# yugabyte/yugabyte-db

Hardware: NVIDIA H100
Metric: compaction GB/s (input bytes merged) (higher is better)
Workload: dtype u8

## Files before the change

yugabyte-db_b200/csrc/engine.cu:

```cuda
#include "engine.h"
#include "host_sst.h"

#include <cuda_runtime.h>
#include <algorithm>
#include <cstdio>
#include <cstring>
#include <chrono>
#include <cstdlib>
#include <mutex>

namespace ybgpu {

#define CUDA_TRY(expr)                                                                      \
  do {                                                                                      \
    cudaError_t _e = (expr);                                                                \
    if (_e != cudaSuccess) {                                                                \
      return FailCuda(#expr, _e);                                                           \
    }                                                                                       \
  } while (0)

struct RunView {
  const uint8_t* data;
  const uint64_t* blk_off;
  const uint32_t* blk_size;
// ... 15 lines not shown
struct JobDev {
  int error;
  uint32_t error_where;
  uint32_t max_ikey_len;
  uint32_t restart_interval[MAX_RUNS];
  unsigned long long in_key_bytes, in_val_bytes;
  unsigned long long n_counted, n_hidden, n_obsolete, n_feed_dropped, n_kept, out_key_bytes, out_val_bytes;
  unsigned long long min_seq, max_seq, n_kept_deletions;
  uint32_t n_rewrites;
  uint32_t n_tiles;
  uint32_t max_tile;
  int ingest_fallback;
  uint32_t n_compressed;
  uint32_t n_lz4;
  uint32_t n_cont_tiles;
  unsigned long long digest;
  unsigned long long verify_fail;
};

struct JobParams {
  int S;
  int k;
  int bottommost;
  uint64_t last_sequence;
  uint32_t largest_len; uint8_t largest[1024];
  uint32_t tile_cap;
  uint32_t H;
  uint32_t M;
  RetentionDev R;
  RangeDev range;
};

struct Desc {
  uint32_t gid;
  uint32_t vlen_out;
  uint16_t klen;
  uint8_t flags;
  uint8_t run;
  uint32_t rewrite_slot;
};

__device__ __forceinline__ void dev_fail(JobDev* J, int code, uint32_t where) {
  if (atomicCAS(&J->error, 0, code) == 0) J->error_where = where;
}

__device__ __forceinline__ uint32_t ldg_u32_unaligned(const uint8_t* p) {
  return static_cast<uint32_t>(p[0]) | (static_cast<uint32_t>(p[1]) << 8) | (static_cast<uint32_t>(p[2]) << 16) |
         (static_cast<uint32_t>(p[3]) << 24);
}

__global__ void __launch_bounds__(256) k_prepass(const RunView* runs, const uint32_t* blk_base , int k, JobDev* J) {
  const int lane = threadIdx.x & 31;
  const uint32_t warp = (blockIdx.x * blockDim.x + threadIdx.x) >> 5;
  const uint32_t nwarps = (gridDim.x * blockDim.x) >> 5;
  unsigned long long key_bytes = 0, val_bytes = 0;
  uint32_t max_klen = 0;
  const uint32_t total_blocks = blk_base[k];
  for (uint32_t gb = warp; gb < total_blocks; gb += nwarps) {
// ... 314 lines not shown
        run.val_off[idx] = boff + p;
        p += vlen;
        idx++;
      }
    }
  }
}

struct PartView {
  const RunView* runs;
  const uint32_t* sample_base;
  uint32_t* pos;
  unsigned long long* bucket_min;
  uint8_t* smode;
  uint32_t n_samples;
  uint32_t n_buckets;
};

constexpr unsigned long long TILE_CONT = 1ull << 63;
constexpr uint32_t SAMPLE_COARSE = 32;
__global__ void __launch_bounds__(256) k_sample_pos(PartView P, const JobParams* prm, JobDev* J, int pass) {
  const int S = prm->S, k = prm->k;
  const uint64_t total = static_cast<uint64_t>(P.n_samples) * k;
  for (uint64_t t = blockIdx.x * static_cast<uint64_t>(blockDim.x) + threadIdx.x; t < total;
       t += static_cast<uint64_t>(gridDim.x) * blockDim.x) {
    const uint32_t s = static_cast<uint32_t>(t / k), r2 = static_cast<uint32_t>(t % k);
    int r = 0;
    while (r + 1 < k && P.sample_base[r + 1] <= s) r++;
    const uint32_t s_local = s - P.sample_base[r];
    if (((s_local % SAMPLE_COARSE) == 0) != (pass == 0)) continue;
    const uint32_t idx = s_local * prm->M;
    const uint8_t* srec = P.runs[r].rec + static_cast<size_t>(idx) * S;
    const int g = group_prefix_len(srec, rec_ulen(srec, S), prm->R.enabled != 0);
    if (g < 0) { dev_fail(J, -g, s); continue; }
    bool inside = false;
    if (idx >= prm->M) {
      const uint8_t* prec = srec - static_cast<size_t>(prm->M) * S;
      inside = rec_ulen(prec, S) >= static_cast<uint32_t>(g) && common_prefix_len(srec, g, prec, g) >= static_cast<uint32_t>(g) &&
               group_prefix_len(prec, rec_ulen(prec, S), prm->R.enabled != 0) == g;
    }
    if (r2 == 0) P.smode[s] = inside ? 1 : 0;
    const RunView& q = P.runs[r2];
    uint32_t lo = 0, hi = q.n_entries;
    if (pass == 1) {
      const uint32_t c0 = s_local - s_local % SAMPLE_COARSE, c1 = c0 + SAMPLE_COARSE;
      lo = P.pos[static_cast<size_t>(P.sample_base[r] + c0) * k + r2];
      if (P.sample_base[r] + c1 < P.sample_base[r + 1]) hi = P.pos[static_cast<size_t>(P.sample_base[r] + c1) * k + r2];
    }
    if (inside) {
      if (r2 == static_cast<uint32_t>(r)) lo = hi = idx;
      while (lo < hi) {
        const uint32_t mid = (lo + hi) >> 1;
        const int c = cmp_records(q.rec + static_cast<size_t>(mid) * S, srec, S);
        if (r2 < static_cast<uint32_t>(r) ? c <= 0 : c < 0) lo = mid + 1; else hi = mid;
      }
    } else {
      while (lo < hi) {
        uint32_t mid = (lo + hi) >> 1;
        const uint8_t* c = q.rec + static_cast<size_t>(mid) * S;
        if (cmp_prefix_vs_key(srec, g, c, rec_ulen(c, S)) > 0) lo = mid + 1; else hi = mid;
      }
    }
    P.pos[static_cast<size_t>(s) * k + r2] = lo;
  }
}

__global__ void __launch_bounds__(256) k_sample_bucket(PartView P, const JobParams* prm) {
  const int k = prm->k;
  for (uint32_t s = blockIdx.x * blockDim.x + threadIdx.x; s < P.n_samples; s += gridDim.x * blockDim.x) {
    unsigned long long rank = 0;
    for (int r = 0; r < k; r++) rank += P.pos[static_cast<size_t>(s) * k + r];
    if (rank == 0) continue;
    uint32_t b = static_cast<uint32_t>(rank / prm->H);
    atomicMin(&P.bucket_min[b], (rank << 28) | s);
  }
}

__device__ __forceinline__ uint32_t block_exclusive_scan(uint32_t v, uint32_t* warp_sums, uint32_t* total) {
  const int lane = threadIdx.x & 31, wid = threadIdx.x >> 5;
  uint32_t x = v;
  for (int o = 1; o < 32; o <<= 1) { uint32_t y = __shfl_up_sync(0xffffffffu, x, o); if (lane >= o) x += y; }
  __syncthreads();
  if (lane == 31) warp_sums[wid] = x;
  __syncthreads();
  if (wid == 0) {
    uint32_t w = lane < (blockDim.x >> 5) ? warp_sums[lane] : 0;
    for (int o = 1; o < 32; o <<= 1) { uint32_t y = __shfl_up_sync(0xffffffffu, w, o); if (lane >= o) w += y; }
    warp_sums[lane] = w;
  }
// ... 41 lines not shown

__global__ void __launch_bounds__(256) k_tile_check(const RunView* runs, const uint32_t* tile_lo, int k, JobDev* J) {
  const uint32_t n_tiles = J->n_tiles;
  uint32_t mx = 0;
  for (uint32_t t = blockIdx.x * blockDim.x + threadIdx.x; t < n_tiles; t += gridDim.x * blockDim.x) {
    uint32_t sz = 0;
    for (int r = 0; r < k; r++) {
      const uint32_t lo = tile_lo[static_cast<size_t>(t) * k + r];
      const uint32_t hi = (t + 1 < n_tiles) ? tile_lo[static_cast<size_t>(t + 1) * k + r] : runs[r].n_entries;
      sz += hi - lo;
    }
    mx = max(mx, sz);
  }
  mx = __reduce_max_sync(0xffffffffu, mx);
  if ((threadIdx.x & 31) == 0 && mx) atomicMax(&J->max_tile, mx);
}

struct MergeView {
  const RunView* runs;
  const uint32_t* tile_lo;
  const unsigned long long* tile_rank;
  Desc* desc;
  ValueRewrite* rewrites;
  uint32_t rewrite_cap;
  uint32_t n_tiles;
  uint16_t* fk16;
  uint32_t* fkh;
  int32_t S, k;
  uint32_t cap;
};
// ... 1235 lines not shown
  }
  const size_t rows_per = std::max<size_t>(1, STAGING_BYTES / row_bytes);
  for (size_t r0 = 0; r0 < rows; r0 += rows_per) {
    const size_t nr = std::min(rows_per, rows - r0);
    const size_t bytes = nr * row_bytes;
    const int grid = src_pitch == row_bytes ? static_cast<int>(std::min<size_t>(64, (bytes + 65535) / 65536)) : static_cast<int>(std::min<size_t>(64, nr));
    k_copy_out<<<std::max(grid, 1), 256, 0, I.stream>>>(I.staging_dev, static_cast<const uint8_t*>(dev_src) + r0 * src_pitch, row_bytes, src_pitch, nr);
    I.readback_launches++;
    CUDA_TRY(cudaGetLastError());
    CUDA_TRY(cudaStreamSynchronize(I.stream));
    memcpy(static_cast<uint8_t*>(host_dst) + r0 * row_bytes, I.staging_host, bytes);
  }
  return YBGPU_OK;
}

ybgpu_status Engine::CheckDeviceError(const char* phase) {
  Impl& I = *impl_;
  if (ybgpu_status s = ReadSmall(&I.hJ, I.dJ, sizeof(JobDev))) return s;
  if (I.hJ.error) {
    char buf[256];
    snprintf(buf, sizeof(buf), "%s (%s, at block/tile %u)", DevErrorName(I.hJ.error), phase, I.hJ.error_where);
    return Fail(DevErrorStatus(I.hJ.error), buf);
  }
  return YBGPU_OK;
}

static cudaError_t EnsureDeviceTables(int device, cudaStream_t stream, int* sms) {
  static std::mutex dev_init_mu;
  static int sm_count[64] = {};
  static bool crc_ready[64] = {};
  std::lock_guard<std::mutex> lock(dev_init_mu);
  cudaError_t e;
  if (!sm_count[device & 63] && (e = cudaDeviceGetAttribute(&sm_count[device & 63], cudaDevAttrMultiProcessorCount, device)) != cudaSuccess) return e;
  if (!crc_ready[device & 63]) {
    k_crc_init<<<1, 256, 0, stream>>>();
    k_crc_init_xpow<<<(CRC_XPOW_TABLE + 256) / 256, 256, 0, stream>>>();
    if ((e = cudaGetLastError()) != cudaSuccess) return e;
    if ((e = cudaStreamSynchronize(stream)) != cudaSuccess) return e;
    crc_ready[device & 63] = true;
// ... 166 lines not shown
    k_scan_blk_counts<<<k, 1024, 0, I.stream>>>(I.dRuns, d_totals);
    launches += 2;
    CUDA_TRY(cudaGetLastError());
    std::vector<uint32_t> cap(k + 1, 0);
    if (ybgpu_status s = ReadSmall(cap.data(), d_totals, 4 * static_cast<size_t>(k))) return s;
    {
      uint64_t cap_total = 0;
      for (int r = 0; r < k; r++) cap_total += cap[r];
      if (cap_total >= (1ull << 32)) return Fail(YBGPU_NOT_SUPPORTED, "more than 2^32 entries in one job: shard the compaction");
    }
    const int S_widest = 16 * ING_NVI + 16;
    const uint32_t sample_max = std::max<uint32_t>(I.hJ.max_ikey_len, 8);
    Sfinal = std::min(S_widest, std::max(32, static_cast<int>(((sample_max - 8 + 16) + 15) & ~15u)));
    IngestView iv{};
    CUDA_TRY(DevAlloc(&I.mem, &iv.ticket, 1));
    CUDA_TRY(cudaFuncSetAttribute(k_ingest, cudaFuncAttributeMaxDynamicSharedMemorySize, static_cast<int>(ING_SMEM)));
    for (int attempt = 0; attempt < 2; attempt++) {
      for (int r = 0; r < k; r++) {
        RunView& rv = I.runs[r];
        CUDA_TRY(DevAlloc(&I.mem, &rv.rec, static_cast<size_t>(cap[r]) * Sfinal + 16));
        if (attempt == 0) {
          CUDA_TRY(DevAlloc(&I.mem, &rv.val_off, static_cast<size_t>(cap[r]) + 1));
          CUDA_TRY(DevAlloc(&I.mem, &rv.val_crc, static_cast<size_t>(cap[r]) + 1));
        }
      }
      if (ybgpu_status us = UploadSmall(I.dRuns, I.runs.data(), sizeof(RunView) * k)) return us;
      CUDA_TRY(cudaMemsetAsync(iv.ticket, 0, 4, I.stream));
      CUDA_TRY(cudaMemsetAsync(&I.dJ->ingest_fallback, 0, sizeof(int), I.stream));
      iv.runs = I.dRuns; iv.blk_base = d_blk_base; iv.totals = d_totals; iv.range = d_range;
      iv.k = k; iv.S = Sfinal; iv.verify = verify_pending ? 1 : 0;
      const int grid = static_cast<int>(std::min<uint64_t>((blk_base[k] + ING_BATCH - 1) / ING_BATCH, static_cast<uint64_t>(sms) * 2));
// ... 103 lines not shown
  hp.M = std::max(1u, std::min(cap / 2, cap - hp.H) / std::max(1, k));
  hp.R.enabled = opt_.retention_enabled;
  hp.R.cutoff_ht = opt_.history_cutoff_ht;
  hp.R.table_ttl_ns = opt_.table_ttl_ns;
  hp.R.cutoff_enc.n = static_cast<uint8_t>(doc_ht_encode(opt_.history_cutoff_ht, 0xffffffffu, hp.R.cutoff_enc.b));
  const uint64_t min_other = opt_.retain_delete_markers_in_major_compaction ? 0 : opt_.other_min_ht;
  hp.R.min_other_enc.n = static_cast<uint8_t>(doc_ht_encode(min_other, 0, hp.R.min_other_enc.b));
  hp.R.ht_min_enc.n = static_cast<uint8_t>(doc_ht_encode(0, 0, hp.R.ht_min_enc.b));
  if (lower_.size() > 255 || upper_.size() > 255) return Fail(YBGPU_NOT_SUPPORTED, "key bounds longer than 255 bytes");
  hp.R.lower_len = static_cast<uint32_t>(lower_.size()); memcpy(hp.R.lower, lower_.data(), lower_.size());
  hp.R.upper_len = static_cast<uint32_t>(upper_.size()); memcpy(hp.R.upper, upper_.data(), upper_.size());
  hp.R.has_cotables_cutoff = opt_.cotables_cutoff_ht != YBGPU_HT_INVALID;
  hp.R.cotables_cutoff_ht = opt_.cotables_cutoff_ht;
  if (hp.R.has_cotables_cutoff) hp.R.cotables_cutoff_enc.n = static_cast<uint8_t>(doc_ht_encode(opt_.cotables_cutoff_ht, 0xffffffffu, hp.R.cotables_cutoff_enc.b));

  if (!opt_.has_largest_user_key) {
    CUDA_TRY(cudaStreamSynchronize(I.stream));
    std::vector<uint8_t> best; bool any = false;
    std::vector<uint8_t> lastrec(static_cast<size_t>(Sfinal) * k);
    for (int r = 0; r < k; r++) {
      if (!I.runs[r].n_entries) continue;
      CUDA_TRY(cudaMemcpyAsync(lastrec.data() + static_cast<size_t>(r) * Sfinal, I.runs[r].rec + static_cast<size_t>(I.runs[r].n_entries - 1) * Sfinal, Sfinal, cudaMemcpyDeviceToHost, I.stream));
    }
    CUDA_TRY(cudaStreamSynchronize(I.stream));
    for (int r = 0; r < k; r++) {
      if (!I.runs[r].n_entries) continue;
      const uint8_t* tmp = lastrec.data() + static_cast<size_t>(r) * Sfinal;
      uint32_t ulen = rec_ulen(tmp, Sfinal);
      std::vector<uint8_t> key(tmp, tmp + ulen);
      if (!any || std::lexicographical_compare(best.begin(), best.end(), key.begin(), key.end())) { best = key; any = true; }
    }
    largest_ = best;
  }
  if (largest_.size() > sizeof(hp.largest)) return Fail(YBGPU_NOT_SUPPORTED, "largest user key too long");
  hp.largest_len = static_cast<uint32_t>(largest_.size());
  memcpy(hp.largest, largest_.data(), largest_.size());
  if (ybgpu_status us = UploadSmall(I.dP, &hp, sizeof(hp))) return us;
  if (ybgpu_status s = CheckDeviceError("decode")) return s;
  tick("decode");
  if (shutdown()) return Fail(YBGPU_SHUTDOWN_IN_PROGRESS, "Database shutdown or Column family drop during compaction");

  if (N == 0) {
    ran_ = true;
    stats_.gpu_kernel_launches = launches;
    return YBGPU_OK;
  }

  uint32_t* d_tile_lo = nullptr; unsigned long long* d_tile_rank = nullptr;
  for (int attempt = 0;; attempt++) {
    std::vector<uint32_t> sample_base(k + 1, 0);
    for (int r = 0; r < k; r++) sample_base[r + 1] = sample_base[r] + (I.runs[r].n_entries + hp.M - 1) / hp.M;
    const uint32_t n_samples = sample_base[k];
    if (n_samples >= (1u << 28)) return Fail(YBGPU_NOT_SUPPORTED, "too many partition samples");
    const uint32_t n_buckets = static_cast<uint32_t>(N / hp.H) + 2;
    PartView pv{};
    uint32_t* d_sample_base = nullptr;
    CUDA_TRY(DevAlloc(&I.mem, &d_sample_base, k + 1));
    CUDA_TRY(DevAlloc(&I.mem, &pv.pos, static_cast<size_t>(n_samples) * k));
    CUDA_TRY(DevAlloc(&I.mem, &pv.smode, n_samples));
    CUDA_TRY(DevAlloc(&I.mem, &pv.bucket_min, n_buckets));
    CUDA_TRY(DevAlloc(&I.mem, &d_tile_lo, static_cast<size_t>(n_buckets + 1) * k));
    CUDA_TRY(DevAlloc(&I.mem, &d_tile_rank, n_buckets + 1));
    if (ybgpu_status us = UploadSmall(d_sample_base, sample_base.data(), 4 * (k + 1))) return us;
    CUDA_TRY(cudaMemsetAsync(pv.bucket_min, 0xff, static_cast<size_t>(n_buckets) * 8, I.stream));
    pv.runs = I.dRuns; pv.sample_base = d_sample_base; pv.n_samples = n_samples; pv.n_buckets = n_buckets;
    k_sample_pos<<<GridFor(static_cast<uint64_t>(n_samples) * k, 256, sms), 256, 0, I.stream>>>(pv, I.dP, I.dJ, 0);
    k_sample_pos<<<GridFor(static_cast<uint64_t>(n_samples) * k, 256, sms), 256, 0, I.stream>>>(pv, I.dP, I.dJ, 1);
    k_sample_bucket<<<GridFor(n_samples, 256, sms), 256, 0, I.stream>>>(pv, I.dP);
    {
      const uint32_t tchunks = (n_buckets + TILE_CHUNK - 1) / TILE_CHUNK;
      uint32_t* d_tpart = nullptr; uint32_t* d_ttotal = nullptr;
      CUDA_TRY(DevAlloc(&I.mem, &d_tpart, tchunks + 1)); CUDA_TRY(DevAlloc(&I.mem, &d_ttotal, 1));
      k_bucket_counts<<<tchunks, 256, 0, I.stream>>>(pv, d_tpart);
      k_scan_u32_single<<<1, 1024, 0, I.stream>>>(d_tpart, tchunks, d_ttotal);
      k_build_tiles<<<tchunks, 256, 0, I.stream>>>(pv, I.dP, d_tpart, d_ttotal, d_tile_lo, d_tile_rank, I.dJ);
      k_tile_check<<<GridFor(n_buckets + 1, 256, sms), 256, 0, I.stream>>>(I.dRuns, d_tile_lo, k, I.dJ);
    }
    launches += 7;
    CUDA_TRY(cudaGetLastError());
    if (ybgpu_status s = CheckDeviceError("partition")) return s;
    if (I.hJ.max_tile <= cap) break;
    if (hp.M <= 1 || attempt >= 4)
      return Fail(YBGPU_NOT_SUPPORTED, "record stride and run count too large for a merge tile");
    hp.M = std::max(1u, hp.M / 2);
    stats_.path_flags |= YBGPU_PATH_PARTITION_RETRY;
    if (ybgpu_status us = UploadSmall(I.dP, &hp, sizeof(hp))) return us;
    CUDA_TRY(cudaMemsetAsync(&I.dJ->max_tile, 0, sizeof(uint32_t), I.stream));
  }
  CUDA_TRY(end_phase());
  tick("partition");
  const uint32_t n_tiles = I.hJ.n_tiles;

  Desc* d_desc = nullptr; ValueRewrite* d_rw = nullptr;
  const uint32_t rewrite_cap = static_cast<uint32_t>(std::min<uint64_t>(N, 1u << 26));
  CUDA_TRY(DevAlloc(&I.mem, &d_desc, N));
  CUDA_TRY(DevAlloc(&I.mem, &d_rw, rewrite_cap));
  MergeView mv{};
  mv.runs = I.dRuns; mv.tile_lo = d_tile_lo; mv.tile_rank = d_tile_rank; mv.desc = d_desc;
  mv.rewrites = d_rw; mv.rewrite_cap = rewrite_cap; mv.n_tiles = n_tiles;
  uint16_t* d_fk16 = nullptr;
  if (opt_.filter_policy != YBGPU_FILTER_NONE && getenv("YBGPU_NO_FK16") == nullptr) CUDA_TRY(DevAlloc(&I.mem, &d_fk16, N));
  mv.fk16 = d_fk16;
  uint32_t* d_fkh = nullptr;
  if (d_fk16) CUDA_TRY(DevAlloc(&I.mem, &d_fkh, N));
  mv.fkh = d_fkh;
  mv.S = Sfinal; mv.k = k; mv.cap = cap;
  const size_t smem = tile_layout::bytes(Sfinal, cap);
  CUDA_TRY(cudaFuncSetAttribute(k_merge_filter, cudaFuncAttributeMaxDynamicSharedMemorySize, static_cast<int>(smem)));
  k_merge_filter<<<n_tiles, MERGE_THREADS, smem, I.stream>>>(mv, I.dP, I.dJ);
  launches++;
  CUDA_TRY(cudaGetLastError());
  CUDA_TRY(end_phase());
  if (ybgpu_status s = CheckDeviceError("merge")) return s;
  tick("merge");
  if (shutdown()) return Fail(YBGPU_SHUTDOWN_IN_PROGRESS, "Database shutdown or Column family drop during compaction");

  I.n_out = I.hJ.n_kept; I.out_key_bytes = I.hJ.out_key_bytes; I.out_val_bytes = I.hJ.out_val_bytes;
  const uint32_t n_chunks = static_cast<uint32_t>((N + EMIT_CHUNK - 1) / EMIT_CHUNK);
  Sums3* d_partial = nullptr;
  CUDA_TRY(DevAlloc(&I.mem, &d_partial, n_chunks + 1));
  I.d_desc = d_desc; I.d_partial = d_partial; I.d_rw = d_rw; I.N = N; I.S = Sfinal; I.n_chunks = n_chunks;
  I.partial_ready = false;
  if (I.n_out != N) { if (ybgpu_status s = EnsureChunkSums()) return s; launches += 2; }
// ... 92 lines not shown
    if (ybgpu_status us = UploadSmall(I.d_block_off + nblocks, &total, 8)) return us;
    I.out_file_len = total;
    CUDA_TRY(DevAlloc(&I.mem, &I.out_file, total + 64));
    {
      const size_t esm = ENC_SMEM_CAP + 32;
      const bool tsp = E.key_encoding == YBGPU_KEY_ENCODING_THREE_SHARED_PARTS;
      const bool v3 = getenv("YBGPU_ENC_V3") != nullptr;
      const uint32_t G = ((4u + 28u + static_cast<uint32_t>(Sfinal) + 32u + 7u) & ~7u) + 4u;
      const size_t v5_smem = 4096 + static_cast<size_t>(ENC5_THREADS) * G;
      const bool v5 = !v3 && getenv("YBGPU_ENC_V4") == nullptr && v5_smem <= 96 * 1024;
      if (!v3) stats_.path_flags |= YBGPU_PATH_ENCODER_V4;
      CUDA_TRY(cudaEventRecord(I.enc_ev[0], I.stream));
      if (v5) {
        stats_.path_flags |= YBGPU_PATH_ENCODER_V5;
        auto kern = tsp ? k_encode_v5<2> : k_encode_v5<1>;
        CUDA_TRY(cudaFuncSetAttribute(kern, cudaFuncAttributeMaxDynamicSharedMemorySize, static_cast<int>(v5_smem)));
        static int occ_cache[2][64] = {};
        int& occ = occ_cache[tsp ? 1 : 0][(Sfinal >> 4) & 63];
        if (!occ) {
          CUDA_TRY(cudaOccupancyMaxActiveBlocksPerMultiprocessor(&occ, kern, ENC5_THREADS, v5_smem));
          if (occ < 1) occ = 1;
        }
        const uint32_t grid = std::min<uint32_t>((nblocks + ENC5_THREADS / 32 - 1) / (ENC5_THREADS / 32), static_cast<uint32_t>(sms) * occ);
        kern<<<grid, ENC5_THREADS, v5_smem, I.stream>>>(E, Sfinal, I.d_block_first, nblocks, I.d_block_off, I.out_file, G);
        launches++;
      } else {
        auto smem_kernel = v3 ? (tsp ? k_encode_smem<2> : k_encode_smem<1>) : (tsp ? k_encode_v4<2> : k_encode_v4<1>);
        auto fused_kernel = tsp ? k_encode_fused<2> : k_encode_fused<1>;
        CUDA_TRY(cudaFuncSetAttribute(smem_kernel, cudaFuncAttributeMaxDynamicSharedMemorySize, static_cast<int>(esm)));
        smem_kernel<<<std::min<uint32_t>(nblocks, sms * 8), ENC_THREADS, esm, I.stream>>>(E, Sfinal, I.d_block_first, nblocks, I.d_block_off, I.out_file);
        launches++;
        if (total_and_max[1] > ENC_SMEM_CAP) {
          fused_kernel<<<std::min<uint32_t>(nblocks, sms * 4), ENC_THREADS, 0, I.stream>>>(E, Sfinal, I.d_block_first, nblocks, I.d_block_off, I.out_file, ENC_SMEM_CAP);
          launches++;
          stats_.path_flags |= YBGPU_PATH_ENCODER_FUSED;
        }
      }
      CUDA_TRY(cudaEventRecord(I.enc_ev[1], I.stream));
      I.enc_timed = true;
    }
    const bool lz4_out = opt_.output_compression == YBGPU_COMPRESSION_LZ4;
    if ((opt_.output_compression == YBGPU_COMPRESSION_SNAPPY || lz4_out) && nblocks) {
      SnapCompView C{};
      C.raw = I.out_file; C.raw_off = I.d_block_off; C.nblocks = nblocks;
// ... 46 lines not shown
      launches += 5;
      stats_.path_flags |= lz4_out ? YBGPU_PATH_LZ4_OUTPUT : YBGPU_PATH_SNAPPY_OUTPUT;
      for (void* dead : {static_cast<void*>(I.out_file), static_cast<void*>(C.comp)}) CUDA_TRY(I.mem.Free(dead, I.stream));
      I.out_file = C.out; I.out_file_len = ftotal; I.d_block_off = d_foff;
    }
    if (E.fk_len) {
      BloomGeometry g{hg.num_lines, hg.num_probes, hg.max_keys, hg.filter_bytes, (hg.filter_bytes + 7u) & ~7u};
      const uint32_t nfb = std::max<uint32_t>(1, (n_keys + g.max_keys - 1) / g.max_keys);
      I.n_filter_blocks = nfb; I.filter_block_bytes = g.block_bytes;
      I.filter_key_stride = static_cast<uint32_t>((max_ikey + 2 + 7) & ~7u);
      CUDA_TRY(DevAlloc(&I.mem, &I.d_filters, static_cast<size_t>(nfb) * g.dev_stride + 16));
      CUDA_TRY(DevAlloc(&I.mem, &I.d_filter_keys, static_cast<size_t>(nfb) * 2 * I.filter_key_stride));
      CUDA_TRY(DevAlloc(&I.mem, &I.d_filter_first, nfb));
      CUDA_TRY(cudaMemsetAsync(I.d_filters, 0, static_cast<size_t>(nfb) * g.dev_stride, I.stream));
      if (n_keys && d_hash) {
        CUDA_TRY(cudaFuncSetAttribute(k_filter_build_smem, cudaFuncAttributeMaxDynamicSharedMemorySize, static_cast<int>(g.dev_stride)));
        const uint32_t resident = std::max<uint32_t>(1, std::min<uint32_t>(2, (200u * 1024u) / (g.dev_stride + 1024u))) * sms;
        const uint32_t parts = std::max<uint32_t>(1, std::min<uint32_t>(8, resident / nfb));
        k_filter_build_smem<<<std::min<uint32_t>(nfb * parts, resident * 4), 1024, g.dev_stride, I.stream>>>(d_hash, n_keys, g, nfb, parts, I.d_filters);
      } else if (n_keys) {
        k_filter_build<<<GridFor(n_keys, 256, sms), 256, 0, I.stream>>>(E, Sfinal, d_new_entry, n_keys, g, I.d_filters);
      }
      k_filter_finish<<<GridFor(static_cast<uint64_t>(nfb) * 2, 256, sms), 256, 0, I.stream>>>(E, Sfinal, d_new_entry, n_keys, g, nfb, I.d_filters,
                                                                                              I.d_filter_keys, I.filter_key_stride, I.d_filter_first);
      launches += 1 + (n_keys ? 1 : 0);
    }
    if (opt_.compute_user_boundary_values && opt_.retention_enabled) {
      const int bgrid = static_cast<int>(std::max<uint64_t>(1, std::min<uint64_t>((n + 255) / 256, static_cast<uint64_t>(sms) * 2)));
      BvCand* d_cand = nullptr;
      CUDA_TRY(DevAlloc(&I.mem, &d_cand, static_cast<size_t>(bgrid) * 2 * BV_MAXC));
      CUDA_TRY(DevAlloc(&I.mem, &I.d_bv, 1));
// ... 408 lines not shown
```

yugabyte-db_b200/csrc/engine.h:

```cpp
#pragma once
#include <mutex>
#include <string>
#include <vector>

#include "../../include/ybgpu_compaction.h"
#include "dev_logic.cuh"

namespace ybgpu {

constexpr int MAX_RUNS = 64;
constexpr char kBudgetExceeded[] = "device memory budget exceeded";

struct MemGroup {
  std::mutex mu;
  uint64_t in_use = 0, peak = 0;
  void Change(int64_t delta) {
    std::lock_guard<std::mutex> l(mu);
    in_use += delta;
    if (in_use > peak) peak = in_use;
  }
};
void JoinMemGroup(ybgpu_job* job, MemGroup* group);

class Engine {
// ... 21 lines not shown
  ybgpu_status FetchFilter(uint8_t* filters, uint8_t* keys, uint32_t* first_entry, uint32_t* block_first);
  ybgpu_status FetchUserValues(ybgpu_user_value* smallest, ybgpu_user_value* largest, uint32_t cap, uint32_t* n);
  ybgpu_status VerifyOutput(ybgpu_output_check* result);
  ybgpu_status VerifySst(const uint8_t* data, uint64_t len, const ybgpu_block_handle* handles, uint64_t nh, int key_encoding,
                         ybgpu_output_check* result);
  const ybgpu_job_options& options() const { return opt_; }
  ybgpu_job_stats& stats();
  const std::string& error() const { return error_; }
  ybgpu_status Fail(ybgpu_status s, const std::string& msg);
  ybgpu_status FailCuda(const char* expr, int e);
  bool ran() const { return ran_; }
  int record_stride() const { return record_stride_; }
  uint32_t num_tiles() const { return num_tiles_; }

 private:
  ybgpu_status CheckDeviceError(const char* phase);
  ybgpu_status CheckBudgetBeforeUpload(uint64_t more);
  ybgpu_status ReadSmall(void* host_dst, const void* dev_src, size_t n);
  ybgpu_status UploadSmall(void* dev_dst, const void* host_src, size_t n);
  ybgpu_status ReadViaMapped(void* host_dst, const void* dev_src, size_t row_bytes, size_t src_pitch, size_t rows);
  ybgpu_status EnsureKvStream();
  ybgpu_status EnsureChunkSums();
  ybgpu_status VerifyTable(const uint8_t* file, uint64_t file_len, const unsigned long long* d_off, const uint32_t* d_size,
                           uint32_t nb, int key_encoding, bool job, ybgpu_output_check* result);
  struct Impl;
  ybgpu_job_options opt_;
  Impl* impl_;
  std::vector<uint8_t> largest_, lower_, upper_, range_lower_, range_upper_;
  ybgpu_job_stats stats_;
  std::string error_;
  bool ran_ = false;
// ... 6 lines not shown
```

Before: 280.3.

## Restructure partition sampling into warp-cooperative kernels and cut host round trips

Replaces the two-pass k_sample_pos plus k_sample_bucket with k_part_coarse and k_part_fine. These assign warps to sample groups, split runs across lanes, and use word-wise comparisons bounded by the coarse positions. The largest-user-key host readback and its stream syncs become a small device kernel. The decode error check is folded into the partition check, and cudaFuncSetAttribute calls are cached per kernel and device. The aim is to shorten the pre-merge front end, at the cost of more complex partition code and coarser error attribution.

```diff
diff --git a/profiles/front_measure.py b/profiles/front_measure.py
--- /dev/null
+++ b/profiles/front_measure.py
@@ -0,0 +1,156 @@
+import argparse
+import collections
+import ctypes
+import importlib
+import json
+import os
+import subprocess
+import sys
+import tempfile
+import time
+
+import numpy as np
+import torch
+
+ROOT = os.path.dirname(os.path.dirname(os.path.abspath(__file__)))
+sys.path[:0] = [ROOT]
+pkg = importlib.import_module("yugabyte-db_b200")
+binding = importlib.import_module("yugabyte-db_b200.binding")
+
+ap = argparse.ArgumentParser()
+ap.add_argument("--rows", type=int, default=40000000)
+ap.add_argument("--steps", type=int, default=3)
+ap.add_argument("--warmup", type=int, default=2)
+ap.add_argument("--host-reps", type=int, default=20, help="jobs timed for the add_input_device split")
+ap.add_argument("--trace-dir", default=None, help="where the chrome trace is written (default: a temporary directory)")
+args = ap.parse_args()
+
+if not torch.cuda.is_available() or pkg.device_count() < 1:
+    raise SystemExit("front_measure.py needs a CUDA device: kernel times cannot be taken without one")
+print(subprocess.run(["nvidia-smi", "--query-gpu=name,power.limit,clocks.max.sm", "--format=csv,noheader"], capture_output=True, text=True).stdout.strip())
+
+cfg = pkg.GenConfig(seed=2, num_rows=args.rows, cols=1, versions=1, num_files=8, value_len=256)
+ssts = pkg.generate_ssts(cfg, max_threads=8)
+handles = [pkg.sst_block_handles(s.meta_view())[:2] for s in ssts]
+print("inputs: %d entries, %.2f GB of data files" % (sum(s.num_entries for s in ssts), sum(s.data_view().size for s in ssts) / 1e9))
+
+dev_files = []
+for s in ssts:
+    v = s.data_view()
+    t = torch.zeros(v.size + 64, dtype=torch.uint8, device="cuda")
+    t[16:16 + v.size].copy_(torch.from_numpy(v))
+    dev_files.append(t)
+torch.cuda.synchronize()
+stream = torch.cuda.current_stream().cuda_stream
+marker = torch.zeros(1, dtype=torch.int32, device="cuda")
+
+
+def new_job():
+    return pkg.GpuCompactionJob(verify_checksums=True, cuda_stream=stream, filter_policy=1)
+
+
+def one_job():
+    job = new_job()
+    for t, s, (off, sz) in zip(dev_files, ssts, handles):
+        job.add_input_device(t.data_ptr() + 16, s.data_view().size, off, sz)
+    st = job.run()
+    marker.add_(1)
+    torch.cuda.synchronize()
+    job.close()
+    return st
+
+
+for _ in range(args.warmup):
+    one_job()
+with torch.profiler.profile(activities=[torch.profiler.ProfilerActivity.CPU, torch.profiler.ProfilerActivity.CUDA]) as prof:
+    stats = [one_job() for _ in range(args.steps)]
+trace_dir = args.trace_dir or tempfile.mkdtemp(prefix="front_measure_")
+os.makedirs(trace_dir, exist_ok=True)
+trace_path = os.path.join(trace_dir, "front_measure_trace.json")
+prof.export_chrome_trace(trace_path)
+
+with open(trace_path) as f:
+    events = json.load(f)["traceEvents"]
+acts = sorted((e for e in events if e.get("ph") == "X" and e.get("cat") in ("kernel", "gpu_memcpy", "gpu_memset")), key=lambda e: e["ts"])
+
+
+def short(e):
+    if e["cat"] != "kernel":
+        return e["cat"] + " " + e["name"].split("(")[0].strip()
+    name = e["name"].split("(")[0]
+    return name.split("::")[-1] if "ybgpu::" in name else name
+
+
+jobs, cur = [], []
+for e in acts:
+    if e["cat"] == "kernel" and "elementwise" in e["name"]:
+        jobs.append(cur)
+        cur = []
+    else:
+        cur.append(e)
+if len(jobs) != args.steps:
+    raise SystemExit("expected %d jobs in the trace, found %d" % (args.steps, len(jobs)))
+
+rows = collections.OrderedDict()
+spans, sums = [], []
+for job in jobs:
+    idx = [i for i, e in enumerate(job) if "k_merge_filter" in e["name"]]
+    if len(idx) != 1:
+        raise SystemExit("a job without exactly one k_merge_filter launch")
+    m = idx[0]
+    prev_end = job[0]["ts"]
+    total = 0.0
+    seen = collections.Counter()
+    for e in job[:m]:
+        name = short(e)
+        seen[name] += 1
+        key = name if e["cat"] != "kernel" or seen[name] == 1 else "%s #%d" % (name, seen[name])
+        r = rows.setdefault(key, [0, 0.0, 0.0])
+        r[0] += 1; r[1] += e["dur"]; r[2] += max(0.0, e["ts"] - prev_end)
+        total += e["dur"]
+        prev_end = max(prev_end, e["ts"] + e["dur"])
+    spans.append(job[m]["ts"] - job[0]["ts"])
+    sums.append(total)
+
+nj = len(jobs)
+print("\nactivities from the start of the job to k_merge_filter, per job (mean of %d profiled jobs; %d entries in, %d launches per job)" % (
+    nj, stats[-1].num_input_records, stats[-1].gpu_kernel_launches))
+print("| activity | launches | total ms | mean us | idle in front, ms |")
+print("|---|---|---|---|---|")
+for name, (cnt, dur, gap) in rows.items():
+    print("| `%s` | %.4g | %.3f | %.1f | %.3f |" % (name, cnt / nj, dur / nj / 1e3, dur / cnt, gap / nj / 1e3))
+print("\nspan from the first activity to the start of k_merge_filter: %s ms" % " ".join("%.3f" % (x / 1e3) for x in spans))
+print("sum of the activities in it:                                 %s ms" % " ".join("%.3f" % (x / 1e3) for x in sums))
+print("difference (launch gaps and host round trips, profiler on):  %s ms" % " ".join("%.3f" % ((a - b) / 1e3) for a, b in zip(spans, sums)))
+ph = stats[-1].phase_seconds
+print("CUDA-event phases of the last job (block scan, ingest, partition, merge, encode; no profiler influence): %s ms" % (
+    " ".join("%.3f" % (x * 1e3) for x in ph[:5])))
+
+L = binding.lib()
+prebuilt = []
+for off, sz in handles:
+    hs = np.zeros((len(off), 2), dtype=np.uint64)
+    hs[:, 0] = off
+    hs[:, 1] = sz
+    prebuilt.append(hs)
+t_bind, t_native = [], []
+for _ in range(args.host_reps):
+    for arm in ("binding", "native"):
+        job = new_job()
+        t0 = time.perf_counter()
+        if arm == "binding":
+            for t, s, (off, sz) in zip(dev_files, ssts, handles):
+                job.add_input_device(t.data_ptr() + 16, s.data_view().size, off, sz)
+        else:
+            for t, s, hs in zip(dev_files, ssts, prebuilt):
+                st = L.ybgpu_job_add_input_device(job.h, t.data_ptr() + 16, s.data_view().size, hs.ctypes.data_as(ctypes.c_void_p), hs.shape[0], 1,
+                                                  binding.HT_INVALID)
+                if st != 0:
+                    raise SystemExit("ybgpu_job_add_input_device failed: %d" % st)
+        t1 = time.perf_counter()
+        (t_bind if arm == "binding" else t_native).append((t1 - t0) * 1e3)
+        torch.cuda.synchronize()
+        job.close()
+med = lambda xs: sorted(xs)[len(xs) // 2]
+print("\nadd_input_device for the job's %d files, host wall (median of %d): binding %.3f ms, native call %.3f ms, binding's own part %.3f ms" % (
+    len(ssts), args.host_reps, med(t_bind), med(t_native), med(t_bind) - med(t_native)))
diff --git a/yugabyte-db_b200/csrc/engine.cu b/yugabyte-db_b200/csrc/engine.cu
--- a/yugabyte-db_b200/csrc/engine.cu
+++ b/yugabyte-db_b200/csrc/engine.cu
@@ -7,6 +7,7 @@
 #include <cstring>
 #include <chrono>
 #include <cstdlib>
+#include <map>
 #include <mutex>
 
 namespace ybgpu {
@@ -53,6 +54,7 @@
   uint32_t n_compressed;
   uint32_t n_lz4;
   uint32_t n_cont_tiles;
+  int error_in_partition;
   unsigned long long digest;
   unsigned long long verify_fail;
 };
@@ -81,6 +83,10 @@
 
 __device__ __forceinline__ void dev_fail(JobDev* J, int code, uint32_t where) {
   if (atomicCAS(&J->error, 0, code) == 0) J->error_where = where;
+}
+
+__device__ __forceinline__ void part_fail(JobDev* J, int code, uint32_t where) {
+  if (atomicCAS(&J->error, 0, code) == 0) { J->error_where = where; J->error_in_partition = 1; }
 }
 
 __device__ __forceinline__ uint32_t ldg_u32_unaligned(const uint8_t* p) {
@@ -425,65 +431,194 @@
   unsigned long long* bucket_min;
   uint8_t* smode;
   uint32_t n_samples;
+  uint32_t n_groups;
+  uint32_t max_run_groups;
   uint32_t n_buckets;
 };
 
 constexpr unsigned long long TILE_CONT = 1ull << 63;
 constexpr uint32_t SAMPLE_COARSE = 32;
-__global__ void __launch_bounds__(256) k_sample_pos(PartView P, const JobParams* prm, JobDev* J, int pass) {
+
+__device__ __forceinline__ int group_run(const uint32_t* sample_base, int k, uint32_t grp, uint32_t* first) {
+  uint32_t g0 = 0;
+  int r = 0;
+  for (;; r++) {
+    const uint32_t n = (sample_base[r + 1] - sample_base[r] + SAMPLE_COARSE - 1) / SAMPLE_COARSE;
+    if (r + 1 >= k || grp < g0 + n) break;
+    g0 += n;
+  }
+  *first = g0;
+  return r;
+}
+
+__device__ __forceinline__ int cmp_probe_vs_rec(const uint8_t* c, const uint8_t* srec, uint32_t slen, int S) {
+  const uint32_t nw = (slen + 7) >> 3;
+  for (uint32_t w = 0; w < nw; w++) {
+    const uint64_t x = ld_u64_aligned(c + 8 * w), y = ld_u64_aligned(srec + 8 * w);
+    if (x != y) return bswap64(x) < bswap64(y) ? -1 : 1;
+  }
+  const uint32_t clen = rec_ulen(c, S);
+  for (uint32_t w = nw; w < ((clen + 7) >> 3); w++)
+    if (ld_u64_aligned(c + 8 * w)) return 1;
+  if (clen != slen) return clen < slen ? -1 : 1;
+  const uint64_t sa = rec_suffix(c, S), sb = rec_suffix(srec, S);
+  return sa > sb ? -1 : (sa < sb ? 1 : 0);
+}
+__device__ __forceinline__ int cmp_prefix_vs_probe(const uint8_t* p, uint32_t g, const uint8_t* c, int S) {
+  const uint32_t nw = (g + 7) >> 3;
+  for (uint32_t w = 0; w < nw; w++) {
+    uint64_t x = ld_u64_aligned(p + 8 * w);
+    const uint32_t valid = g - 8 * w;
+    if (valid < 8) x &= (1ull << (8 * valid)) - 1;
+    const uint64_t y = ld_u64_aligned(c + 8 * w);
+    if (x != y) return bswap64(x) < bswap64(y) ? -1 : 1;
+  }
+  const uint32_t clen = rec_ulen(c, S);
+  for (uint32_t w = nw; w < ((clen + 7) >> 3); w++)
+    if (ld_u64_aligned(c + 8 * w)) return -1;
+  return g < clen ? -1 : (g > clen ? 1 : 0);
+}
+
+__device__ __forceinline__ uint32_t splitter_pos(const RunView& q, int r2, int r, const uint8_t* srec, int g, bool inside, uint32_t idx,
+                                                 uint32_t lo, uint32_t hi, int S) {
+  hi = min(hi, q.n_entries);
+  lo = min(lo, hi);
+  if (r2 == r) {
+    if (inside) return idx;
+    hi = min(hi, idx);
+  }
+  if (inside) {
+    const uint32_t slen = rec_ulen(srec, S);
+    while (lo < hi) {
+      const uint32_t mid = (lo + hi) >> 1;
+      const int c = cmp_probe_vs_rec(q.rec + static_cast<size_t>(mid) * S, srec, slen, S);
+      if (r2 < r ? c <= 0 : c < 0) lo = mid + 1; else hi = mid;
+    }
+  } else {
+    while (lo < hi) {
+      const uint32_t mid = (lo + hi) >> 1;
+      if (cmp_prefix_vs_probe(srec, g, q.rec + static_cast<size_t>(mid) * S, S) > 0) lo = mid + 1; else hi = mid;
+    }
+  }
+  return lo;
+}
+
+__global__ void __launch_bounds__(256) k_part_coarse(PartView P, const JobParams* prm, JobDev* J, int kp) {
   const int S = prm->S, k = prm->k;
-  const uint64_t total = static_cast<uint64_t>(P.n_samples) * k;
-  for (uint64_t t = blockIdx.x * static_cast<uint64_t>(blockDim.x) + threadIdx.x; t < total;
-       t += static_cast<uint64_t>(gridDim.x) * blockDim.x) {
-    const uint32_t s = static_cast<uint32_t>(t / k), r2 = static_cast<uint32_t>(t % k);
-    int r = 0;
-    while (r + 1 < k && P.sample_base[r + 1] <= s) r++;
-    const uint32_t s_local = s - P.sample_base[r];
-    if (((s_local % SAMPLE_COARSE) == 0) != (pass == 0)) continue;
-    const uint32_t idx = s_local * prm->M;
-    const uint8_t* srec = P.runs[r].rec + static_cast<size_t>(idx) * S;
-    const int g = group_prefix_len(srec, rec_ulen(srec, S), prm->R.enabled != 0);
-    if (g < 0) { dev_fail(J, -g, s); continue; }
-    bool inside = false;
-    if (idx >= prm->M) {
-      const uint8_t* prec = srec - static_cast<size_t>(prm->M) * S;
-      inside = rec_ulen(prec, S) >= static_cast<uint32_t>(g) && common_prefix_len(srec, g, prec, g) >= static_cast<uint32_t>(g) &&
-               group_prefix_len(prec, rec_ulen(prec, S), prm->R.enabled != 0) == g;
-    }
-    if (r2 == 0) P.smode[s] = inside ? 1 : 0;
-    const RunView& q = P.runs[r2];
-    uint32_t lo = 0, hi = q.n_entries;
-    if (pass == 1) {
-      const uint32_t c0 = s_local - s_local % SAMPLE_COARSE, c1 = c0 + SAMPLE_COARSE;
-      lo = P.pos[static_cast<size_t>(P.sample_base[r] + c0) * k + r2];
-      if (P.sample_base[r] + c1 < P.sample_base[r + 1]) hi = P.pos[static_cast<size_t>(P.sample_base[r] + c1) * k + r2];
-    }
-    if (inside) {
-      if (r2 == static_cast<uint32_t>(r)) lo = hi = idx;
-      while (lo < hi) {
-        const uint32_t mid = (lo + hi) >> 1;
-        const int c = cmp_records(q.rec + static_cast<size_t>(mid) * S, srec, S);
-        if (r2 < static_cast<uint32_t>(r) ? c <= 0 : c < 0) lo = mid + 1; else hi = mid;
-      }
-    } else {
-      while (lo < hi) {
-        uint32_t mid = (lo + hi) >> 1;
-        const uint8_t* c = q.rec + static_cast<size_t>(mid) * S;
-        if (cmp_prefix_vs_key(srec, g, c, rec_ulen(c, S)) > 0) lo = mid + 1; else hi = mid;
-      }
-    }
-    P.pos[static_cast<size_t>(s) * k + r2] = lo;
-  }
-}
-
-__global__ void __launch_bounds__(256) k_sample_bucket(PartView P, const JobParams* prm) {
-  const int k = prm->k;
-  for (uint32_t s = blockIdx.x * blockDim.x + threadIdx.x; s < P.n_samples; s += gridDim.x * blockDim.x) {
-    unsigned long long rank = 0;
-    for (int r = 0; r < k; r++) rank += P.pos[static_cast<size_t>(s) * k + r];
-    if (rank == 0) continue;
-    uint32_t b = static_cast<uint32_t>(rank / prm->H);
-    atomicMin(&P.bucket_min[b], (rank << 28) | s);
+  const uint32_t M = prm->M;
+  const bool retention = prm->R.enabled != 0;
+  const int lane = threadIdx.x & 31, j = lane & (kp - 1);
+  const uint32_t sub = lane / kp, per_step = 32 / kp;
+  const uint32_t nwarps = (gridDim.x * blockDim.x) >> 5;
+  for (uint32_t base = ((blockIdx.x * blockDim.x + threadIdx.x) >> 5) * 32; base < P.n_groups; base += nwarps * 32) {
+    int my_g = 0;
+    bool my_inside = false;
+    const uint8_t* my_rec = nullptr;
+    bool has_prev = false;
+    if (base + lane < P.n_groups) {
+      uint32_t g0;
+      const int r = group_run(P.sample_base, k, base + lane, &g0);
+      const uint32_t idx = (base + lane - g0) * SAMPLE_COARSE * M;
+      my_rec = P.runs[r].rec + static_cast<size_t>(idx) * S;
+      has_prev = idx >= M;
+      if (has_prev) {
+        const uint8_t* prec = my_rec - static_cast<size_t>(M) * S;
+        my_g = group_prefix_len(prec, rec_ulen(prec, S), retention);
+      }
+    }
+    const int prev_g = my_g;
+    if (my_rec) {
+      my_g = group_prefix_len(my_rec, rec_ulen(my_rec, S), retention);
+      const uint8_t* prec = my_rec - static_cast<size_t>(M) * S;
+      my_inside = my_g >= 0 && has_prev && rec_ulen(prec, S) >= static_cast<uint32_t>(my_g) &&
+                  common_prefix_len(my_rec, my_g, prec, my_g) >= static_cast<uint32_t>(my_g) && prev_g == my_g;
+    }
+    for (uint32_t m0 = 0; m0 < 32; m0 += per_step) {
+      const uint32_t m = m0 + sub, grp = base + m;
+      const bool active = grp < P.n_groups;
+      const int g = __shfl_sync(0xffffffffu, my_g, m);
+      const bool inside = __shfl_sync(0xffffffffu, my_inside ? 1 : 0, m) != 0;
+      if (!active) continue;
+      uint32_t g0;
+      const int r = group_run(P.sample_base, k, grp, &g0);
+      const uint32_t s_local = (grp - g0) * SAMPLE_COARSE, idx = s_local * M, s = P.sample_base[r] + s_local;
+      if (g < 0) { if (j == 0) part_fail(J, -g, s); continue; }
+      if (j == 0) P.smode[s] = inside ? 1 : 0;
+      const uint8_t* srec = P.runs[r].rec + static_cast<size_t>(idx) * S;
+      for (int r2 = j; r2 < k; r2 += kp)
+        P.pos[static_cast<size_t>(s) * k + r2] = splitter_pos(P.runs[r2], r2, r, srec, g, inside, idx, 0, P.runs[r2].n_entries, S);
+    }
+  }
+}
+
+__global__ void __launch_bounds__(256) k_part_fine(PartView P, const JobParams* prm, JobDev* J, int kp) {
+  const int S = prm->S, k = prm->k;
+  const uint32_t M = prm->M, H = prm->H;
+  const bool retention = prm->R.enabled != 0;
+  const int lane = threadIdx.x & 31, j = lane & (kp - 1);
+  const uint32_t sub = lane / kp, per_step = 32 / kp;
+  const uint32_t nwarps = (gridDim.x * blockDim.x) >> 5;
+  const uint32_t n_slots = P.max_run_groups * k;
+  for (uint32_t slot = (blockIdx.x * blockDim.x + threadIdx.x) >> 5; slot < n_slots; slot += nwarps) {
+    const int r = static_cast<int>(slot % k);
+    const uint32_t t = slot / k;
+    const uint32_t sb = P.sample_base[r], ns = P.sample_base[r + 1] - sb;
+    const uint32_t ng = (ns + SAMPLE_COARSE - 1) / SAMPLE_COARSE;
+    const uint32_t c = static_cast<uint32_t>(static_cast<uint64_t>(t) * ng / P.max_run_groups);
+    if ((t && static_cast<uint64_t>(t - 1) * ng / P.max_run_groups == c) || c >= ng) continue;
+    const uint32_t c0 = c * SAMPLE_COARSE, n_in = min(SAMPLE_COARSE, ns - c0);
+    const uint32_t* next = c0 + SAMPLE_COARSE < ns ? P.pos + static_cast<size_t>(sb + c0 + SAMPLE_COARSE) * k : nullptr;
+    uint32_t* row0 = P.pos + static_cast<size_t>(sb + c0) * k;
+    const uint8_t* rec0 = P.runs[r].rec;
+    int my_g = 0;
+    bool my_inside = false;
+    {
+      const uint8_t* srec = rec0 + static_cast<size_t>(c0 + lane) * M * S;
+      if (static_cast<uint32_t>(lane) < n_in) my_g = group_prefix_len(srec, rec_ulen(srec, S), retention);
+      const int prev_g = __shfl_up_sync(0xffffffffu, my_g, 1);
+      if (lane > 0 && static_cast<uint32_t>(lane) < n_in && my_g >= 0) {
+        const uint8_t* prec = srec - static_cast<size_t>(M) * S;
+        my_inside = rec_ulen(prec, S) >= static_cast<uint32_t>(my_g) &&
+                    common_prefix_len(srec, my_g, prec, my_g) >= static_cast<uint32_t>(my_g) && prev_g == my_g;
+      }
+    }
+    if (lane == 0) {
+      unsigned long long rank = 0;
+      for (int r2 = 0; r2 < k; r2++) rank += row0[r2];
+      const unsigned long long b = rank / H;
+      if (rank && b < P.n_buckets) atomicMin(&P.bucket_min[b], (rank << 28) | (sb + c0));
+    }
+    for (uint32_t h = SAMPLE_COARSE / 2; h; h >>= 1) {
+      const uint32_t cnt = SAMPLE_COARSE / (2 * h);
+      for (uint32_t m0 = 0; m0 < cnt; m0 += per_step) {
+        const uint32_t i = h * (2 * (m0 + sub) + 1);
+        const bool active = m0 + sub < cnt && i < n_in;
+        const uint32_t s = sb + c0 + i, idx = (c0 + i) * M;
+        const uint8_t* srec = rec0 + static_cast<size_t>(idx) * S;
+        const int g = __shfl_sync(0xffffffffu, my_g, active ? i : 0);
+        const bool inside = __shfl_sync(0xffffffffu, my_inside ? 1 : 0, active ? i : 0) != 0;
+        unsigned long long rank = 0;
+        if (active && g >= 0) {
+          if (j == 0) P.smode[s] = inside ? 1 : 0;
+          const uint32_t* lo_row = row0 + static_cast<size_t>(i - h) * k;
+          const uint32_t* hi_row = i + h < n_in ? row0 + static_cast<size_t>(i + h) * k : (i + h == SAMPLE_COARSE ? next : nullptr);
+          for (int r2 = j; r2 < k; r2 += kp) {
+            const RunView& q = P.runs[r2];
+            const uint32_t p = splitter_pos(q, r2, r, srec, g, inside, idx, lo_row[r2], hi_row ? hi_row[r2] : q.n_entries, S);
+            row0[static_cast<size_t>(i) * k + r2] = p;
+            rank += p;
+          }
+        } else if (active && j == 0) {
+          part_fail(J, -g, s);
+        }
+        for (int o = kp >> 1; o; o >>= 1) rank += __shfl_xor_sync(0xffffffffu, rank, o, kp);
+        if (active && g >= 0 && j == 0 && rank) {
+          const unsigned long long b = rank / H;
+          if (b < P.n_buckets) atomicMin(&P.bucket_min[b], (rank << 28) | s);
+        }
+      }
+      __syncwarp();
+    }
   }
 }
 
@@ -555,6 +690,19 @@
   }
   mx = __reduce_max_sync(0xffffffffu, mx);
   if ((threadIdx.x & 31) == 0 && mx) atomicMax(&J->max_tile, mx);
+}
+
+__global__ void __launch_bounds__(32) k_largest_key(const RunView* runs, int k, int S, JobParams* prm) {
+  const uint8_t* best = nullptr;
+  uint32_t best_len = 0;
+  for (int r = 0; r < k; r++) {
+    if (!runs[r].n_entries) continue;
+    const uint8_t* rec = runs[r].rec + static_cast<size_t>(runs[r].n_entries - 1) * S;
+    const uint32_t len = rec_ulen(rec, S);
+    if (!best || cmp_user_keys(best, best_len, rec, len) < 0) { best = rec; best_len = len; }
+  }
+  for (uint32_t i = threadIdx.x; i < best_len; i += 32) prm->largest[i] = best[i];
+  if (threadIdx.x == 0) prm->largest_len = best_len;
 }
 
 struct MergeView {
@@ -1820,15 +1968,27 @@
   return YBGPU_OK;
 }
 
-ybgpu_status Engine::CheckDeviceError(const char* phase) {
+ybgpu_status Engine::CheckDeviceError(const char* phase, const char* partition_phase) {
   Impl& I = *impl_;
   if (ybgpu_status s = ReadSmall(&I.hJ, I.dJ, sizeof(JobDev))) return s;
   if (I.hJ.error) {
+    if (partition_phase && I.hJ.error_in_partition) phase = partition_phase;
     char buf[256];
     snprintf(buf, sizeof(buf), "%s (%s, at block/tile %u)", DevErrorName(I.hJ.error), phase, I.hJ.error_where);
     return Fail(DevErrorStatus(I.hJ.error), buf);
   }
   return YBGPU_OK;
+}
+
+static cudaError_t AllowDynamicSmem(const void* kernel, int device, size_t bytes) {
+  static std::mutex mu;
+  static std::map<std::pair<const void*, int>, size_t> allowed;
+  std::lock_guard<std::mutex> lock(mu);
+  size_t& cur = allowed[{kernel, device}];
+  if (bytes <= cur) return cudaSuccess;
+  const cudaError_t e = cudaFuncSetAttribute(kernel, cudaFuncAttributeMaxDynamicSharedMemorySize, static_cast<int>(bytes));
+  if (e == cudaSuccess) cur = bytes;
+  return e;
 }
 
 static cudaError_t EnsureDeviceTables(int device, cudaStream_t stream, int* sms) {
@@ -2025,7 +2185,7 @@
     Sfinal = std::min(S_widest, std::max(32, static_cast<int>(((sample_max - 8 + 16) + 15) & ~15u)));
     IngestView iv{};
     CUDA_TRY(DevAlloc(&I.mem, &iv.ticket, 1));
-    CUDA_TRY(cudaFuncSetAttribute(k_ingest, cudaFuncAttributeMaxDynamicSharedMemorySize, static_cast<int>(ING_SMEM)));
+    CUDA_TRY(AllowDynamicSmem(reinterpret_cast<const void*>(k_ingest), opt_.device, ING_SMEM));
     for (int attempt = 0; attempt < 2; attempt++) {
       for (int r = 0; r < k; r++) {
         RunView& rv = I.runs[r];
@@ -2159,37 +2319,23 @@
   hp.R.cotables_cutoff_ht = opt_.cotables_cutoff_ht;
   if (hp.R.has_cotables_cutoff) hp.R.cotables_cutoff_enc.n = static_cast<uint8_t>(doc_ht_encode(opt_.cotables_cutoff_ht, 0xffffffffu, hp.R.cotables_cutoff_enc.b));
 
-  if (!opt_.has_largest_user_key) {
-    CUDA_TRY(cudaStreamSynchronize(I.stream));
-    std::vector<uint8_t> best; bool any = false;
-    std::vector<uint8_t> lastrec(static_cast<size_t>(Sfinal) * k);
-    for (int r = 0; r < k; r++) {
-      if (!I.runs[r].n_entries) continue;
-      CUDA_TRY(cudaMemcpyAsync(lastrec.data() + static_cast<size_t>(r) * Sfinal, I.runs[r].rec + static_cast<size_t>(I.runs[r].n_entries - 1) * Sfinal, Sfinal, cudaMemcpyDeviceToHost, I.stream));
-    }
-    CUDA_TRY(cudaStreamSynchronize(I.stream));
-    for (int r = 0; r < k; r++) {
-      if (!I.runs[r].n_entries) continue;
-      const uint8_t* tmp = lastrec.data() + static_cast<size_t>(r) * Sfinal;
-      uint32_t ulen = rec_ulen(tmp, Sfinal);
-      std::vector<uint8_t> key(tmp, tmp + ulen);
-      if (!any || std::lexicographical_compare(best.begin(), best.end(), key.begin(), key.end())) { best = key; any = true; }
-    }
-    largest_ = best;
-  }
   if (largest_.size() > sizeof(hp.largest)) return Fail(YBGPU_NOT_SUPPORTED, "largest user key too long");
   hp.largest_len = static_cast<uint32_t>(largest_.size());
   memcpy(hp.largest, largest_.data(), largest_.size());
   if (ybgpu_status us = UploadSmall(I.dP, &hp, sizeof(hp))) return us;
-  if (ybgpu_status s = CheckDeviceError("decode")) return s;
-  tick("decode");
-  if (shutdown()) return Fail(YBGPU_SHUTDOWN_IN_PROGRESS, "Database shutdown or Column family drop during compaction");
-
   if (N == 0) {
+    if (ybgpu_status s = CheckDeviceError("decode")) return s;
     ran_ = true;
     stats_.gpu_kernel_launches = launches;
     return YBGPU_OK;
   }
+  if (!opt_.has_largest_user_key) {
+    k_largest_key<<<1, 32, 0, I.stream>>>(I.dRuns, k, Sfinal, I.dP);
+    launches++;
+    CUDA_TRY(cudaGetLastError());
+  }
+  tick("decode");
+  if (shutdown()) return Fail(YBGPU_SHUTDOWN_IN_PROGRESS, "Database shutdown or Column family drop during compaction");
 
   uint32_t* d_tile_lo = nullptr; unsigned long long* d_tile_rank = nullptr;
   for (int attempt = 0;; attempt++) {
@@ -2209,9 +2355,17 @@
     if (ybgpu_status us = UploadSmall(d_sample_base, sample_base.data(), 4 * (k + 1))) return us;
     CUDA_TRY(cudaMemsetAsync(pv.bucket_min, 0xff, static_cast<size_t>(n_buckets) * 8, I.stream));
     pv.runs = I.dRuns; pv.sample_base = d_sample_base; pv.n_samples = n_samples; pv.n_buckets = n_buckets;
-    k_sample_pos<<<GridFor(static_cast<uint64_t>(n_samples) * k, 256, sms), 256, 0, I.stream>>>(pv, I.dP, I.dJ, 0);
-    k_sample_pos<<<GridFor(static_cast<uint64_t>(n_samples) * k, 256, sms), 256, 0, I.stream>>>(pv, I.dP, I.dJ, 1);
-    k_sample_bucket<<<GridFor(n_samples, 256, sms), 256, 0, I.stream>>>(pv, I.dP);
+    uint32_t n_groups = 0, max_run_groups = 0;
+    for (int r = 0; r < k; r++) {
+      const uint32_t ng = (sample_base[r + 1] - sample_base[r] + SAMPLE_COARSE - 1) / SAMPLE_COARSE;
+      n_groups += ng;
+      max_run_groups = std::max(max_run_groups, ng);
+    }
+    pv.n_groups = n_groups; pv.max_run_groups = max_run_groups;
+    int kp = 1;
+    while (kp < std::min(k, 32)) kp <<= 1;
+    k_part_coarse<<<GridFor(n_groups, 256, sms), 256, 0, I.stream>>>(pv, I.dP, I.dJ, kp);
+    k_part_fine<<<GridFor(static_cast<uint64_t>(max_run_groups) * k * 32, 256, sms), 256, 0, I.stream>>>(pv, I.dP, I.dJ, kp);
     {
       const uint32_t tchunks = (n_buckets + TILE_CHUNK - 1) / TILE_CHUNK;
       uint32_t* d_tpart = nullptr; uint32_t* d_ttotal = nullptr;
@@ -2221,15 +2375,15 @@
       k_build_tiles<<<tchunks, 256, 0, I.stream>>>(pv, I.dP, d_tpart, d_ttotal, d_tile_lo, d_tile_rank, I.dJ);
       k_tile_check<<<GridFor(n_buckets + 1, 256, sms), 256, 0, I.stream>>>(I.dRuns, d_tile_lo, k, I.dJ);
     }
-    launches += 7;
+    launches += 6;
     CUDA_TRY(cudaGetLastError());
-    if (ybgpu_status s = CheckDeviceError("partition")) return s;
+    if (ybgpu_status s = CheckDeviceError("decode", "partition")) return s;
     if (I.hJ.max_tile <= cap) break;
     if (hp.M <= 1 || attempt >= 4)
       return Fail(YBGPU_NOT_SUPPORTED, "record stride and run count too large for a merge tile");
     hp.M = std::max(1u, hp.M / 2);
     stats_.path_flags |= YBGPU_PATH_PARTITION_RETRY;
-    if (ybgpu_status us = UploadSmall(I.dP, &hp, sizeof(hp))) return us;
+    if (ybgpu_status us = UploadSmall(&I.dP->M, &hp.M, sizeof(hp.M))) return us;
     CUDA_TRY(cudaMemsetAsync(&I.dJ->max_tile, 0, sizeof(uint32_t), I.stream));
   }
   CUDA_TRY(end_phase());
@@ -2251,7 +2405,7 @@
   mv.fkh = d_fkh;
   mv.S = Sfinal; mv.k = k; mv.cap = cap;
   const size_t smem = tile_layout::bytes(Sfinal, cap);
-  CUDA_TRY(cudaFuncSetAttribute(k_merge_filter, cudaFuncAttributeMaxDynamicSharedMemorySize, static_cast<int>(smem)));
+  CUDA_TRY(AllowDynamicSmem(reinterpret_cast<const void*>(k_merge_filter), opt_.device, smem));
   k_merge_filter<<<n_tiles, MERGE_THREADS, smem, I.stream>>>(mv, I.dP, I.dJ);
   launches++;
   CUDA_TRY(cudaGetLastError());
@@ -2374,7 +2528,7 @@
       if (v5) {
         stats_.path_flags |= YBGPU_PATH_ENCODER_V5;
         auto kern = tsp ? k_encode_v5<2> : k_encode_v5<1>;
-        CUDA_TRY(cudaFuncSetAttribute(kern, cudaFuncAttributeMaxDynamicSharedMemorySize, static_cast<int>(v5_smem)));
+        CUDA_TRY(AllowDynamicSmem(reinterpret_cast<const void*>(kern), opt_.device, v5_smem));
         static int occ_cache[2][64] = {};
         int& occ = occ_cache[tsp ? 1 : 0][(Sfinal >> 4) & 63];
         if (!occ) {
@@ -2387,7 +2541,7 @@
       } else {
         auto smem_kernel = v3 ? (tsp ? k_encode_smem<2> : k_encode_smem<1>) : (tsp ? k_encode_v4<2> : k_encode_v4<1>);
         auto fused_kernel = tsp ? k_encode_fused<2> : k_encode_fused<1>;
-        CUDA_TRY(cudaFuncSetAttribute(smem_kernel, cudaFuncAttributeMaxDynamicSharedMemorySize, static_cast<int>(esm)));
+        CUDA_TRY(AllowDynamicSmem(reinterpret_cast<const void*>(smem_kernel), opt_.device, esm));
         smem_kernel<<<std::min<uint32_t>(nblocks, sms * 8), ENC_THREADS, esm, I.stream>>>(E, Sfinal, I.d_block_first, nblocks, I.d_block_off, I.out_file);
         launches++;
         if (total_and_max[1] > ENC_SMEM_CAP) {
@@ -2464,7 +2618,7 @@
       CUDA_TRY(DevAlloc(&I.mem, &I.d_filter_first, nfb));
       CUDA_TRY(cudaMemsetAsync(I.d_filters, 0, static_cast<size_t>(nfb) * g.dev_stride, I.stream));
       if (n_keys && d_hash) {
-        CUDA_TRY(cudaFuncSetAttribute(k_filter_build_smem, cudaFuncAttributeMaxDynamicSharedMemorySize, static_cast<int>(g.dev_stride)));
+        CUDA_TRY(AllowDynamicSmem(reinterpret_cast<const void*>(k_filter_build_smem), opt_.device, g.dev_stride));
         const uint32_t resident = std::max<uint32_t>(1, std::min<uint32_t>(2, (200u * 1024u) / (g.dev_stride + 1024u))) * sms;
         const uint32_t parts = std::max<uint32_t>(1, std::min<uint32_t>(8, resident / nfb));
         k_filter_build_smem<<<std::min<uint32_t>(nfb * parts, resident * 4), 1024, g.dev_stride, I.stream>>>(d_hash, n_keys, g, nfb, parts, I.d_filters);
diff --git a/yugabyte-db_b200/csrc/engine.h b/yugabyte-db_b200/csrc/engine.h
--- a/yugabyte-db_b200/csrc/engine.h
+++ b/yugabyte-db_b200/csrc/engine.h
@@ -59,7 +59,7 @@
   uint32_t num_tiles() const { return num_tiles_; }
 
  private:
-  ybgpu_status CheckDeviceError(const char* phase);
+  ybgpu_status CheckDeviceError(const char* phase, const char* partition_phase = nullptr);
   ybgpu_status CheckBudgetBeforeUpload(uint64_t more);
   ybgpu_status ReadSmall(void* host_dst, const void* dev_src, size_t n);
   ybgpu_status UploadSmall(void* dev_dst, const void* host_src, size_t n);
```

Result: no change. 281.6 (median of 6 runs) (+0.5%).
